# rahulaggarwal965/vslam

Measured on AMD Instinct MI355X. Metric: frame-pairs/sec (extract+match+RANSAC) @1280×720, 2k kp, 4096 hyp; 1/2/4/8 GPU, higher is better.
Workload: dtype u8/f32/f64; 1 GPU; C3: 1280x720, 2000 keypoints, 4096 hypotheses, batch 256 pairs per GPU, SURVEY 8(d) data: rotation + parallax, sub-pixel resampling, 40-45 % outlier matches; pairs_per_gpu=256, batches_in_flight=4

## Files before the change

vslam_amd/csrc/ransac_count.hip:

```cpp
#include "ransac_prune_tile.h"
#include "ransac_residual.h"

namespace {
using namespace vs_ransac;

constexpr int kCntHyps = 128;
constexpr int kCntWaves = 8;
constexpr int kCntQueue = 320;
constexpr int kCntLdsMatches = 4096;
constexpr int kScreenMatches = 128;
constexpr int kScreenHyps = 128;
constexpr int kRankThreads = 512;
constexpr int kPilotHyps = kRankThreads / 64;
constexpr int kCandMax = 8;
constexpr float kCntTinyDD = 0x1p-120f;
constexpr int kFcmpOGT = 2, kFcmpOLT = 4, kFcmpULT = 12;
constexpr int kCntRec = 12;
typedef __attribute__((address_space(3))) volatile uint32_t cnt_queue_t;
static_assert(VSLAM_MAX_KP <= 65536, "queue words keep the match index in 16 bits");

__host__ __device__ constexpr int cnt_pad(int n) { return (n + 255) & ~255; }
constexpr int kHeadUncertified = kVsHeadUncertified;
__device__ __forceinline__ float cnt_sum_rel(int adds) { return fmaxf(0x1p-18f, (float)(13 + adds) * 0x1p-24f); }

// ... 197 lines not shown
}

__global__ __launch_bounds__(kRankThreads) void ransac_rank_kernel(
    const float *__restrict__ xy1, const float *__restrict__ xy2, const int32_t *__restrict__ pairs,
    const int32_t *__restrict__ m_arr, int min_m, int kp_stride, int kp_pad, int hyp, float threshold,
    const float *__restrict__ hypF, int32_t *__restrict__ cbound, float *__restrict__ rk, float *__restrict__ cmax,
    unsigned long long *__restrict__ sfloor) {
    const int b = blockIdx.x, tid = threadIdx.x, lane = tid & 63;
    const int wave = __builtin_amdgcn_readfirstlane(tid >> 6);
    const int m = min(m_arr[b], kp_stride);
    if (m < min_m) return;
    __shared__ double s_psum[kPilotHyps];
    __shared__ unsigned long long s_bits[kPilotHyps][VSLAM_MAX_KP / 64];
    __shared__ int s_hist[kPilotHyps][kPilotHyps + 1], s_off[kPilotHyps][kPilotHyps + 1], s_pcount[kPilotHyps];
    const float2 *P1 = reinterpret_cast<const float2 *>(xy1) + (size_t)b * kp_stride;
    const float2 *P2 = reinterpret_cast<const float2 *>(xy2) + (size_t)b * kp_stride;
    const int2 *PR = reinterpret_cast<const int2 *>(pairs) + (size_t)b * kp_stride;
    const int npil = min(kPilotHyps, hyp);
    const int G = (m + 63) >> 6;

    if (wave < npil) {
        const int h = (int)(((long long)hyp * wave) / npil);
        ResidualF R;
        const float *src = hypF + ((size_t)b * hyp + h) * 9;
#pragma unroll
        for (int j = 0; j < 9; j++) R.f[j] = src[j];
        residual_prepare(R);
        int count = 0;
        double esum = 0;
        float c1 = 0.f, c2 = 0.f;
        for (int g0 = 0; g0 < G; g0 += 4) {
            int2 pr[4];
            float2 a[4], c[4];
#pragma unroll
            for (int u = 0; u < 4; u++) pr[u] = PR[min((g0 + u) * 64 + lane, m - 1)];
#pragma unroll
            for (int u = 0; u < 4; u++) {
                a[u] = P1[pr[u].x];
                c[u] = P2[pr[u].y];
            }
#pragma unroll
            for (int u = 0; u < 4; u++) {
                const float e = residual_e(R, make_float4(a[u].x, a[u].y, c[u].x, c[u].y), (double)c[u].x, (double)c[u].y);
                const unsigned long long in = __ballot((g0 + u) * 64 + lane < m && e <= threshold);
                count += __popcll(in);
                if ((g0 + u) * 64 + lane < m) esum += (double)e;
                if (lane == 0 && g0 + u < G) s_bits[wave][g0 + u] = in;
                c1 = fmaxf(c1, fmaxf(fabsf(a[u].x), fabsf(a[u].y)));
                c2 = fmaxf(c2, fmaxf(fabsf(c[u].x), fabsf(c[u].y)));
            }
        }
#pragma unroll
        for (int off = 32; off > 0; off >>= 1) esum += __shfl_xor(esum, off, 64);
        if (lane == 0) {
            s_pcount[wave] = count;
            s_psum[wave] = esum;
        }
        if (wave == 0) {
#pragma unroll
            for (int off = 32; off > 0; off >>= 1) {
                c1 = fmaxf(c1, __shfl_xor(c1, off, 64));
                c2 = fmaxf(c2, __shfl_xor(c2, off, 64));
            }
            if (lane == 0) {
                cmax[2 * b] = c1;
                cmax[2 * b + 1] = c2;
            }
        }
    }
    __syncthreads();

    const int gpw = (G + kPilotHyps - 1) / kPilotHyps;
    const int g_lo = min(G, wave * gpw), g_hi = min(G, g_lo + gpw);
    int hist[kPilotHyps + 1];
#pragma unroll
    for (int v = 0; v <= kPilotHyps; v++) hist[v] = 0;
    for (int g = g_lo; g < g_hi; g++) {
        const bool valid = g * 64 + lane < m;
        int key = 0;
        for (int w = 0; w < npil; w++) key += (int)((~s_bits[w][g] >> lane) & 1ull);
#pragma unroll
        for (int v = 0; v <= kPilotHyps; v++) hist[v] += __popcll(__ballot(valid && key == v));
    }
    if (lane == 0) {
#pragma unroll
        for (int v = 0; v <= kPilotHyps; v++) s_hist[wave][v] = hist[v];
    }
    __syncthreads();
    if (tid == 0) {
        int best = 0;
        for (int w = 0; w < npil; w++) best = max(best, s_pcount[w]);
        cbound[b] = best;
        if (sfloor) {
            double fl = -INFINITY;
            bool any_nan = false;
            for (int w = 0; w < npil; w++)
                if (s_pcount[w] == best) {
                    any_nan = any_nan || !(s_psum[w] == s_psum[w]);
                    if (s_psum[w] > fl) fl = s_psum[w];
                }
            const bool valid = best > 0 && !any_nan && fl > 0 && fl < 0x1p120;
            sfloor[b] = valid ? ((unsigned long long)(uint32_t)best << 32) | (unsigned long long)__float_as_uint((float)(fl * (1.0 - 0x1p-20))) : 0ull;
        }
        int run = 0;
        for (int v = kPilotHyps; v >= 0; v--)
            for (int w = 0; w < kPilotHyps; w++) {
                s_off[w][v] = run;
                run += s_hist[w][v];
            }
    }
    __syncthreads();
    int off[kPilotHyps + 1];
#pragma unroll
    for (int v = 0; v <= kPilotHyps; v++) off[v] = s_off[wave][v];
    float *r = rk + (size_t)b * 4 * kp_pad;
    for (int g = g_lo; g < g_hi; g++) {
        const int i = g * 64 + lane;
        const bool valid = i < m;
        int key = 0;
        for (int w = 0; w < npil; w++) key += (int)((~s_bits[w][g] >> lane) & 1ull);
        int pos = 0;
#pragma unroll
        for (int v = 0; v <= kPilotHyps; v++) {
            const unsigned long long bal = __ballot(valid && key == v);
            const int rank = (int)__builtin_amdgcn_mbcnt_hi((uint32_t)(bal >> 32), __builtin_amdgcn_mbcnt_lo((uint32_t)bal, 0u));
            if (key == v) pos = off[v] + rank;
            off[v] += __popcll(bal);
        }
        if (valid) {
            const int2 pr = PR[i];
            const float2 a = P1[pr.x], c = P2[pr.y];
            r[pos] = a.x;
            r[kp_pad + pos] = a.y;
            r[2 * kp_pad + pos] = c.x;
            r[3 * kp_pad + pos] = c.y;
        }
    }
    const int mpad = cnt_pad(m);
    if (m + tid < mpad) {
        const int2 pr = PR[m - 1];
        const float2 a = P1[pr.x], c = P2[pr.y];
        r[m + tid] = a.x;
        r[kp_pad + m + tid] = a.y;
        r[2 * kp_pad + m + tid] = c.x;
        r[3 * kp_pad + m + tid] = c.y;
    }
}

#ifdef VSLAM_EXPERIMENTS
#define VS_SCREEN_ROUTE_PARAM , int32_t *__restrict__ route_out
#else
#define VS_SCREEN_ROUTE_PARAM
#endif
__global__ __launch_bounds__(256) __attribute__((amdgpu_waves_per_eu(7, 7))) void ransac_screen_kernel(
    const float *__restrict__ rk, int kp_pad, const int32_t *__restrict__ m_arr, int min_m, int kp_stride, int hyp,
    float threshold, const float *__restrict__ hypF, const float *__restrict__ cmax, const int32_t *__restrict__ cbound,
    int32_t *__restrict__ pot0, int2 *__restrict__ head, float splus, int route VS_SCREEN_ROUTE_PARAM) {
    const int b = blockIdx.y, tid = threadIdx.x, lane = tid & 63;
    const int wave = __builtin_amdgcn_readfirstlane(tid >> 6);
    const int hbase = blockIdx.x * kScreenHyps;
    const int m = min(m_arr[b], kp_stride);
    const int bound_pilots = cbound[b];
#ifdef VSLAM_EXPERIMENTS
    if (route_out && blockIdx.x == 0 && tid == 0)
        route_out[b] = m < min_m ? -1 : (vs_head_on_certificate(m, bound_pilots, min(m, kScreenMatches), route) ? 1 : 0);
#endif
    if (m < min_m) return;
    if (vs_head_on_certificate(m, bound_pilots, min(m, kScreenMatches), route)) {
        static_assert(kScreenHyps == vs_prune::kPruneWaves * vs_prune::kPruneHyps && kScreenMatches <= vs_prune::kHeadTiles * vs_prune::kPruneTile,
                      "a wave of the screen is a wave of the prune tile");
        if (hbase + wave * 32 < hyp)
            vs_prune::head_on_certificate(rk, kp_pad, b, m, min(m, kScreenMatches), hbase + wave * 32, hyp, threshold, splus, hypF, cmax, pot0, head);
        return;
    }
    __shared__ __align__(16) float s_rec[kScreenHyps * kCntRec];
    if (tid < kScreenHyps) {
        const float *src = hypF + ((size_t)b * hyp + min(hbase + tid, hyp - 1)) * 9;
        float f[9];
#pragma unroll
        for (int k = 0; k < 9; k++) f[k] = src[k];
        const CntBand B = cnt_band(f, cmax[2 * b], cmax[2 * b + 1], threshold);
        cnt_store_record(s_rec + tid * kCntRec, f, B);
    }
    const int n0 = min(m, kScreenMatches);
    const float *r = rk + (size_t)b * 4 * kp_pad;
    const float2 x1 = *reinterpret_cast<const float2 *>(r + 2 * lane);
    const float2 y1 = *reinterpret_cast<const float2 *>(r + kp_pad + 2 * lane);
    const float2 x2 = *reinterpret_cast<const float2 *>(r + 2 * kp_pad + 2 * lane);
    const float2 y2 = *reinterpret_cast<const float2 *>(r + 3 * kp_pad + 2 * lane);
    v2f X1, Y1, X2, Y2;
    X1.x = x1.x; X1.y = x1.y; Y1.x = y1.x; Y1.y = y1.y;
    X2.x = x2.x; X2.y = x2.y; Y2.x = y2.x; Y2.y = y2.y;
    const unsigned long long va = __ballot(2 * lane < n0), vb = __ballot(2 * lane + 1 < n0);
    __syncthreads();
    int mine = 0;
    float mine_sum = 0.f;
    const bool odd1 = (lane & 1) != 0, odd2 = (lane & 2) != 0;
    const bool in_a = 2 * lane < n0, in_b = 2 * lane + 1 < n0;
    constexpr int kU = 4;
    static_assert(kU == 4, "the head sums are reduced four hypotheses at a time");
    for (int j = 0; j < 32; j += kU) {
        CntRec R[kU];
        v2f dd[kU], g[kU];
#pragma unroll
        for (int u = 0; u < kU; u++) cnt_load_record(R[u], s_rec, wave * 32 + j + u);
#pragma unroll
        for (int u = 0; u < kU; u++) g[u] = cnt_cheap(R[u], X1, Y1, X2, Y2, dd[u]);
        bool any_alive = false;
#pragma unroll
        for (int u = 0; u < kU; u++) {
            const unsigned long long oa = __builtin_amdgcn_fcmpf(g[u].x, R[u].hi, kFcmpOGT), ob = __builtin_amdgcn_fcmpf(g[u].y, R[u].hi, kFcmpOGT);
            const unsigned long long ia = __builtin_amdgcn_fcmpf(g[u].x, R[u].lo, kFcmpOLT), ib = __builtin_amdgcn_fcmpf(g[u].y, R[u].lo, kFcmpOLT);
            int p = __popcll(va & ~oa) + __popcll(vb & ~ob);
            int c = __popcll(va & ia) + __popcll(vb & ib);
            if (__builtin_amdgcn_fcmpf(fminf(dd[u].x, dd[u].y), kCntTinyDD, kFcmpULT) != 0ull) {
                p = n0;
                c = 0xFF;
            }
            mine = lane == j + u ? (p | (c << 8)) : mine;
            any_alive = any_alive || p + (m - n0) >= bound_pilots;
        }
        if (!any_alive) continue;
        float v[kU];
#pragma unroll
        for (int u = 0; u < kU; u++) v[u] = (in_a ? g[u].x : 0.f) + (in_b ? g[u].y : 0.f);
        const int z = 0;
        const float k01 = odd1 ? v[1] : v[0], t01 = odd1 ? v[0] : v[1], k23 = odd1 ? v[3] : v[2], t23 = odd1 ? v[2] : v[3];
        const float r01 = k01 + __int_as_float(__builtin_amdgcn_update_dpp(z, __float_as_int(t01), 0xB1, 0xF, 0xF, false));
        const float r23 = k23 + __int_as_float(__builtin_amdgcn_update_dpp(z, __float_as_int(t23), 0xB1, 0xF, 0xF, false));
        const float kk = odd2 ? r23 : r01, tt = odd2 ? r01 : r23;
        float r = kk + __int_as_float(__builtin_amdgcn_update_dpp(z, __float_as_int(tt), 0x4E, 0xF, 0xF, false));
        r += __int_as_float(__builtin_amdgcn_update_dpp(z, __float_as_int(r), 0x124, 0xF, 0xF, false));
        r += __int_as_float(__builtin_amdgcn_update_dpp(z, __float_as_int(r), 0x128, 0xF, 0xF, false));
        r += __shfl_xor(r, 16, 64);
        r += __shfl_xor(r, 32, 64);
        mine_sum = (lane >> 2) == (j >> 2) ? r : mine_sum;
    }
    const int h = hbase + wave * 32 + lane;
    if (lane < 32 && h < hyp) {
        const int c = mine >> 8;
        pot0[(size_t)b * hyp + h] = mine & 0xFF;
        head[(size_t)b * hyp + h] = make_int2(c == 0xFF ? kHeadUncertified : c, __float_as_int(mine_sum));
    }
}

__global__ __launch_bounds__(64 * kCandMax) void ransac_cand_kernel(
    const float *__restrict__ rk, int kp_pad, const int32_t *__restrict__ m_arr, int min_m, int kp_stride, int hyp,
    float threshold, const float *__restrict__ hypF, const int32_t *__restrict__ pot0, int by_sum,
    int32_t *__restrict__ cbound, unsigned long long *__restrict__ sfloor) {
    const int b = blockIdx.x, tid = threadIdx.x, lane = tid & 63;
    const int wave = __builtin_amdgcn_readfirstlane(tid >> 6);
    const int m = min(m_arr[b], kp_stride);
    if (m < min_m) return;
    __shared__ int s_max[kCandMax], s_l0[kCandMax][kCandMax], s_l1[kCandMax][kCandMax], s_n0[kCandMax], s_n1[kCandMax];
    __shared__ int s_cand[kCandMax], s_nc;
    const int32_t *P = pot0 + (size_t)b * hyp;
    int mx = -1;
    for (int i = tid; i < hyp; i += 64 * kCandMax) mx = max(mx, P[i]);
#pragma unroll
    for (int off = 32; off > 0; off >>= 1) mx = max(mx, __shfl_xor(mx, off, 64));
    if (lane == 0) s_max[wave] = mx;
    __syncthreads();
    mx = s_max[0];
    for (int w = 1; w < kCandMax; w++) mx = max(mx, s_max[w]);
    const int per = (hyp + kCandMax - 1) / kCandMax;
    const int lo = min(hyp, wave * per), hi = min(hyp, lo + per);
    int n0 = 0, n1 = 0;
    __shared__ int s_samp[kCandMax][32];
    int nsamp = 0;
    for (int i0 = lo; i0 < hi && ((by_sum && nsamp < 32) || n0 < kCandMax || n1 < kCandMax); i0 += 64) {
        const int i = i0 + lane;
        const int v = i < hi ? P[i] : -2;
        unsigned long long b0 = __ballot(v == mx), b1 = __ballot(v == mx - 1);
        if (by_sum) {
            const int rs = nsamp + __popcll(b0 & ((1ull << lane) - 1ull));
            if (v == mx && rs < 32) s_samp[wave][rs] = i;
            nsamp = min(32, nsamp + (int)__popcll(b0));
        }
        const int r0 = n0 + __popcll(b0 & ((1ull << lane) - 1ull)), r1 = n1 + __popcll(b1 & ((1ull << lane) - 1ull));
        if (v == mx && r0 < kCandMax) s_l0[wave][r0] = i;
        if (v == mx - 1 && r1 < kCandMax) s_l1[wave][r1] = i;
        n0 = min(kCandMax, n0 + __popcll(b0));
        n1 = min(kCandMax, n1 + __popcll(b1));
    }
    if (by_sum && nsamp > 1) {
        const int n128 = min(m, kScreenMatches);
        const float *r = rk + (size_t)b * 4 * kp_pad;
        const float2 x1 = *reinterpret_cast<const float2 *>(r + 2 * lane), y1 = *reinterpret_cast<const float2 *>(r + kp_pad + 2 * lane);
        const float2 x2 = *reinterpret_cast<const float2 *>(r + 2 * kp_pad + 2 * lane), y2 = *reinterpret_cast<const float2 *>(r + 3 * kp_pad + 2 * lane);
        v2f X1, Y1, X2, Y2;
        X1.x = x1.x; X1.y = x1.y; Y1.x = y1.x; Y1.y = y1.y;
        X2.x = x2.x; X2.y = x2.y; Y2.x = y2.x; Y2.y = y2.y;
        float fl[9];
        {
            const int hs = s_samp[wave][lane < nsamp ? lane : 0];
            const float *src = hypF + ((size_t)b * hyp + hs) * 9;
#pragma unroll
            for (int k = 0; k < 9; k++) fl[k] = src[k];
        }
        float best_s = -INFINITY;
        int best_i = -1;
        for (int j = 0; j < nsamp; j++) {
            CntRec R;
#pragma unroll
            for (int k = 0; k < 9; k++) R.f[k] = __int_as_float(__builtin_amdgcn_readlane(__float_as_int(fl[k]), j));
            v2f dd;
            const v2f g = cnt_cheap(R, X1, Y1, X2, Y2, dd);
            const float part = wave_sum_to_lane63((2 * lane < n128 ? g.x : 0.f) + (2 * lane + 1 < n128 ? g.y : 0.f));
            const float tot = __int_as_float(__builtin_amdgcn_readlane(__float_as_int(part), 63));
            if (tot > best_s) {
                best_s = tot;
                best_i = s_samp[wave][j];
            }
        }
        if (lane == 0 && best_i >= 0 && n0 > 0) {
            const int old = s_l0[wave][0];
            for (int k = 1; k < n0; k++)
                if (s_l0[wave][k] == best_i) s_l0[wave][k] = old;
            s_l0[wave][0] = best_i;
        }
    }
    if (lane == 0) {
        s_n0[wave] = n0;
        s_n1[wave] = n1;
    }
// ... 158 lines not shown
            if (lane == 0) knext = atomicAdd(&s_next, 1);
            int hh;
            {
                int kk = k, w = 0;
                while (w + 1 < kListWaves && kk >= s_nlist[w]) kk -= s_nlist[w++];
                hh = s_list[w * 64 + kk];
            }
            bound = max(bound, *(__attribute__((address_space(3))) const volatile int *)&s_bound);
            CntRec R;
            cnt_load_record(R, s_rec, hh);
            const int word = ZERO ? 0 : s_state[hh] >> 2;
            const int head_cnt = ZERO ? 0 : *(__attribute__((address_space(3))) const volatile int *)&s_cnt[hh];
            float head_sum = ZERO ? 0.f : s_part[hh];
            int cnt = 0, pot = word & 0xFFFF, seen = org;
            bool dropped = false, unk = false;
            v2f acc;
            acc.x = 0.f;
            acc.y = 0.f;
            for (int s = 0;; s++) {
                if (s >= nsub && (ZERO || s > nsub || !(word & kHeadMine))) break;
                const bool hd = !ZERO && s == nsub;
                const int pot_walk = pot;
                const int ix = (hd ? 0 : org + s * 256) + 4 * lane;
                const int il = min(ix, mpad - 4);
                const float4 X1 = *reinterpret_cast<const float4 *>(cx1 + il), Y1 = *reinterpret_cast<const float4 *>(cy1 + il);
                const float4 X2 = *reinterpret_cast<const float4 *>(cx2 + il), Y2 = *reinterpret_cast<const float4 *>(cy2 + il);
                if (hd || (s == nsub - 1 && part)) {
                    cnt_sub_block<true>(R, X1, Y1, X2, Y2, ix, hh, lane, hd ? n0 : m, cnt, q, qn, acc, s_unk, pot, unk);
                    seen += hd ? 0 : (m - org) & 255;
                } else {
                    cnt_sub_block<false>(R, X1, Y1, X2, Y2, ix, hh, lane, m, cnt, q, qn, acc, s_unk, pot, unk);
                    seen += 256;
                }
                while (qn >= 64) {
                    cnt_drain(q, qn - 64, 64, lane, s_rec, s_cnt, cx1, cy1, cx2, cy2, threshold);
                    qn -= 64;
                }
                if (hd) {
                    head_sum = 0.f;
                    pot = pot_walk;
                    break;
                }
                if (pot + (m - seen) < bound) {
                    dropped = true;
                    break;
                }
                if (seen < m && bound == floor_count && pot + (m - seen) == bound && !unk && R.beta >= 0.f && !(word & kHeadNoSum)) {
                    const float S = head_sum + __int_as_float(__builtin_amdgcn_readlane(__float_as_int(wave_sum_to_lane63(acc.x + acc.y)), 63));
                    const float ns = (float)seen;
                    const float err = (2.02f * R.beta * sqrtf(ns * S) + ns * R.beta * R.beta + sum_rel * S) * 1.0001f;
                    const float upper = ((S + err) + threshold * (float)(m - seen)) * 1.0001f;
                    if (upper < floor_sum * 0.9999f) {
                        dropped = true;
                        break;
                    }
                }
            }
            if (dropped) {
#ifdef VSLAM_EXPERIMENTS
                if (lane == 0) s_state[hh] = 2 | (seen << 2);
#else
                if (lane == 0) s_state[hh] = 2;
#endif
            } else {
                const float part_sum = head_sum + wave_sum_to_lane63(acc.x + acc.y);
                bool beaten = false;
                if (bound == floor_count && pot == bound && !unk && R.beta >= 0.f) {
                    const float S = __int_as_float(__builtin_amdgcn_readlane(__float_as_int(part_sum), 63));
                    const float ns = (float)m;
                    const float err = (2.02f * R.beta * sqrtf(ns * S) + ns * R.beta * R.beta + sum_rel * S) * 1.0001f;
                    beaten = (S + err) * 1.0001f < floor_sum * 0.9999f;
                }
                if (lane == 63) s_part[hh] = part_sum;
                const int certain = head_cnt + cnt;
                if (beaten) {
#ifdef VSLAM_EXPERIMENTS
                    if (lane == 0) s_state[hh] = 2 | (seen << 2);
#else
                    if (lane == 0) s_state[hh] = 2;
#endif
                } else if (lane == 0) {
                    if (cnt) atomicAdd(&s_cnt[hh], cnt);
                    if (certain > bound) {
                        atomicMax(&s_bound, certain);
                        atomicMax(&cbound[b], certain);
                    }
                }
                if (!beaten) bound = max(bound, certain);
            }
            k = __builtin_amdgcn_readfirstlane(knext);
        }
        if (qn > 0) cnt_drain(q, 0, qn, lane, s_rec, s_cnt, cx1, cy1, cx2, cy2, threshold);
    }
    __syncthreads();
    if (tid < nh) {
        const int st = s_state[tid] & 3;
        hyp_count[out] = st == 1 ? s_cnt[tid] : -1;
        int nan_bits = 0x7FC00000;
#ifdef VSLAM_EXPERIMENTS
        if (exit_payload && st != 1) nan_bits |= st == 2 ? min(s_state[tid] >> 2, 0x3FFFFF) : 0x3FFFFF;
#endif
        hyp_sum[out] = __int_as_float(nan_bits);
        const float S = st == 1 ? s_part[tid] : 0.f;
        float err = INFINITY;
        if (st == 1 && my_ok && !s_unk[tid]) {
            const double Sd = (double)S;
            const double rel = (double)cnt_sum_rel(2 * ((m - (ZERO ? 0 : n0) + 255) >> 8) + 9);
            err = (float)((2.02 * my_beta * sqrt((double)m * Sd) + (double)m * my_beta * my_beta + rel * Sd) * (1.0 + 0x1p-20));
        }
        reinterpret_cast<float2 *>(approx)[out] = make_float2(S, err);
    }
}

}

int vs_launch_ransac_count(vslam_ctx *ctx, const float *xy1, const float *xy2, const int32_t *pairs, const int32_t *m,
                           const float *hypF, int batch, int kp_stride, int hyp, float threshold, int32_t *hyp_count,
                           float *hyp_sum, float *approx) {
    const int min_m = ctx->ransac_min_matches;
    int rc;
    int32_t *cbound = nullptr, *pot0 = nullptr;
    float *rk = nullptr, *cmax = nullptr;
    const int kp_pad = cnt_pad(kp_stride);
    if ((rc = vs_arena_get(ctx, "ransac.cbound", sizeof(int32_t) * (size_t)batch, (void **)&cbound))) return rc;
    unsigned long long *sfloor = nullptr;
    if ((rc = vs_arena_get(ctx, "ransac.sfloor", sizeof(unsigned long long) * (size_t)batch, (void **)&sfloor))) return rc;
    static const bool no_sum_rule = VS_EXPERIMENT_ENV("VSLAM_RANSAC_NO_SUM_RULE") != nullptr;
    const bool from_zero = VS_EXPERIMENT_ENV("VSLAM_RANSAC_COUNT_FROM_ZERO") != nullptr;
#ifdef VSLAM_EXPERIMENTS
    const int exit_payload = VS_EXPERIMENT_ENV("VSLAM_RANSAC_COUNT_EXIT_PAYLOAD") != nullptr ? 1 : 0;
#endif
    int2 *head = nullptr;
    if ((rc = vs_arena_get(ctx, "ransac.head", sizeof(int2) * (size_t)batch * hyp, (void **)&head))) return rc;
    const unsigned long long *use_floor = no_sum_rule ? nullptr : sfloor;
    if ((rc = vs_arena_get(ctx, "ransac.pot0", sizeof(int32_t) * (size_t)batch * hyp, (void **)&pot0))) return rc;
    if ((rc = vs_arena_get(ctx, "ransac.rk", sizeof(float) * 4 * (size_t)kp_pad * batch, (void **)&rk))) return rc;
    if ((rc = vs_arena_get(ctx, "ransac.cmax", sizeof(float) * 2 * (size_t)batch, (void **)&cmax))) return rc;
    {
        VsProfScope ps(ctx, "ransac_rank_kernel");
        ransac_rank_kernel<<<batch, kRankThreads, 0, ctx->stream>>>(xy1, xy2, pairs, m, min_m, kp_stride, kp_pad, hyp, threshold, hypF,
                                                                    cbound, rk, cmax, sfloor);
    }
    int route = -1;
    if (const char *e = VS_EXPERIMENT_ENV("VSLAM_RANSAC_HEAD_ROUTE")) route = atoi(e) ? 1 : 0;
#ifdef VSLAM_EXPERIMENTS
    int32_t *route_out = nullptr, *pot0_out = nullptr;
    if ((rc = vs_arena_get(ctx, "ransac.head_route", sizeof(int32_t) * (size_t)batch, (void **)&route_out))) return rc;
    if ((rc = vs_arena_get(ctx, "ransac.head_pot0", sizeof(int32_t) * (size_t)batch * hyp, (void **)&pot0_out))) return rc;
#endif
    {
        VsProfScope ps(ctx, "ransac_screen_kernel");
        dim3 grid(vs_div_up(hyp, kScreenHyps), batch);
#ifdef VSLAM_EXPERIMENTS
        ransac_screen_kernel<<<grid, 256, 0, ctx->stream>>>(rk, kp_pad, m, min_m, kp_stride, hyp, threshold, hypF, cmax, cbound, pot0, head,
                                                            pc_splus(threshold), route, route_out);
#else
        ransac_screen_kernel<<<grid, 256, 0, ctx->stream>>>(rk, kp_pad, m, min_m, kp_stride, hyp, threshold, hypF, cmax, cbound, pot0, head,
                                                            pc_splus(threshold), route);
#endif
    }
#ifdef VSLAM_EXPERIMENTS
    VS_HIP(ctx, hipMemcpyAsync(pot0_out, pot0, sizeof(int32_t) * (size_t)batch * hyp, hipMemcpyDeviceToDevice, ctx->stream));
#endif
    {
        VsProfScope ps(ctx, "ransac_cand_kernel");
        ransac_cand_kernel<<<batch, 64 * kCandMax, 0, ctx->stream>>>(rk, kp_pad, m, min_m, kp_stride, hyp, threshold, hypF, pot0,
                                                                     no_sum_rule ? 0 : 1, cbound, sfloor);
    }
    if ((rc = vs_launch_ransac_prune(ctx, rk, kp_pad, m, min_m, kp_stride, hyp, threshold, hypF, cmax, cbound, pot0, batch, kScreenMatches)))
        return rc;
    if (int arc = vs_aux_job_point(ctx, 4)) return arc;
    {
        VsProfScope ps(ctx, "ransac_count_kernel");
        const bool lds = kp_pad <= kCntLdsMatches;
        const size_t dyn = (lds ? sizeof(float) * 4 * (size_t)kp_pad : 0) + sizeof(uint32_t) * kCntQueue * kCntWaves;
        const size_t dyn_max = sizeof(float) * 4 * kCntLdsMatches + sizeof(uint32_t) * kCntQueue * kCntWaves;
        dim3 grid(vs_div_up(hyp, kCntHyps), batch);
#ifdef VSLAM_EXPERIMENTS
        if (from_zero) {
            if (dyn > 32 * 1024 && (rc = vs_allow_dynamic_lds(ctx, ransac_count_kernel<true, true>, "ransac_count_from_zero", dyn_max)))
                return rc;
            if (lds)
                ransac_count_kernel<true, true><<<grid, 64 * kCntWaves, dyn, ctx->stream>>>(
                    rk, kp_pad, m, min_m, kp_stride, hyp, threshold, hypF, pot0, head, cmax, hyp_count, hyp_sum, approx, cbound,
                    use_floor VS_CNT_PAYLOAD_ARG);
            else
                ransac_count_kernel<false, true><<<grid, 64 * kCntWaves, dyn, ctx->stream>>>(
                    rk, kp_pad, m, min_m, kp_stride, hyp, threshold, hypF, pot0, head, cmax, hyp_count, hyp_sum, approx, cbound,
                    use_floor VS_CNT_PAYLOAD_ARG);
            return VSLAM_OK;
        }
#endif
        (void)from_zero;
        if (dyn > 32 * 1024 &&
            (rc = vs_allow_dynamic_lds(ctx, ransac_count_kernel<true, false>, "ransac_count", dyn_max)))
            return rc;
        if (lds)
            ransac_count_kernel<true, false><<<grid, 64 * kCntWaves, dyn, ctx->stream>>>(
                rk, kp_pad, m, min_m, kp_stride, hyp, threshold, hypF, pot0, head, cmax, hyp_count, hyp_sum, approx, cbound,
                    use_floor VS_CNT_PAYLOAD_ARG);
        else
            ransac_count_kernel<false, false><<<grid, 64 * kCntWaves, dyn, ctx->stream>>>(
                rk, kp_pad, m, min_m, kp_stride, hyp, threshold, hypF, pot0, head, cmax, hyp_count, hyp_sum, approx, cbound,
                    use_floor VS_CNT_PAYLOAD_ARG);
    }
    return VSLAM_OK;
}
```

vslam_amd/csrc/ransac_prune.hip:

```cpp
#include "ransac_prune_tile.h"

namespace {
using namespace vs_prune;

constexpr int kPruneStep = 2;

#ifdef VSLAM_EXPERIMENTS
#define VS_PRUNE_X_PARAM , int32_t *__restrict__ x_out
#else
#define VS_PRUNE_X_PARAM
#endif

__global__ __launch_bounds__(64 * kPruneWaves) void ransac_prune_mfma_kernel(
    const float *__restrict__ rk, int kp_pad, const int32_t *__restrict__ m_arr, int min_m, int kp_stride, int hyp, float threshold,
    float splus, const float *__restrict__ hypF, const float *__restrict__ cmax, const int32_t *__restrict__ cbound, int32_t *__restrict__ pot0,
    int n_head, int gate VS_PRUNE_X_PARAM) {
    const int b = blockIdx.y, lane = threadIdx.x & 63, col = lane & 31;
    const bool half = lane >= 32;
    const int wave = __builtin_amdgcn_readfirstlane(threadIdx.x >> 6);
    const int m = min(m_arr[b], kp_stride);
    const int bound = cbound[b];
    if (m < min_m) return;
    const int n0 = min(m, n_head);
    const int hbase = (blockIdx.x * kPruneWaves + wave) * kPruneHyps;
    if (m <= n0 || hbase >= hyp) return;
    if (gate && m - bound + 1 <= n0) return;

    const int h = hbase + col;
    const size_t hi = (size_t)b * hyp + min(h, hyp - 1);
    const int behind = m - n0;
    const int lim = pot0[hi] + behind - bound;
    bool live0 = h < hyp && lim >= 0 && lim < behind;
    if (__ballot(live0) == 0ull) return;
    float f[9];
#pragma unroll
    for (int k = 0; k < 9; k++) f[k] = hypF[hi * 9 + k];
    const float c = pc_margin(f, cmax[2 * b], cmax[2 * b + 1], threshold, splus);
    live0 = live0 && c < INFINITY;
    if (__ballot(live0) == 0ull) return;
    const PruneA A = prune_operands(f, half);
    float cr[16];
#pragma unroll
    for (int r = 0; r < 16; r++) cr[r] = __shfl(c, half ? prune_row(r, 1) : prune_row(r, 0), 64);

    const float *r1 = rk + (size_t)b * 4 * kp_pad, *r2 = r1 + kp_pad, *r3 = r2 + kp_pad, *r4 = r3 + kp_pad;
    int X[kPruneHyps], L[kPruneHyps];
#pragma unroll
    for (int i = 0; i < kPruneHyps; i++) {
        X[i] = 0;
        L[i] = __builtin_amdgcn_readlane(live0 ? lim : -1, i);
    }
    const int end = m;
    for (int base = n0; base < end; base += kPruneStep * kPruneTile) {
        float x1[kPruneStep], y1[kPruneStep], x2[kPruneStep], y2[kPruneStep];
#pragma unroll
        for (int t = 0; t < kPruneStep; t++) {
            const int j = min(base + t * kPruneTile + col, m - 1);
            x1[t] = r1[j];
            y1[t] = r2[j];
            x2[t] = r3[j];
            y2[t] = r4[j];
        }
#pragma unroll
        for (int t = 0; t < kPruneStep; t++) {
            v16f n, a0;
            prune_tile(A, half, x1[t], y1[t], x2[t], y2[t], n, a0);
            const unsigned long long valid = __ballot(base + t * kPruneTile + col < end);
#pragma unroll
            for (int r = 0; r < 16; r++) {
                const unsigned long long miss =
                    __builtin_amdgcn_fcmpf(fabsf(n[r]), fmaf(splus, fabsf(a0[r]), cr[r]), kPruneOGT) & valid;
                X[prune_row(r, 0)] += __popc((uint32_t)miss);
                X[prune_row(r, 1)] += __popc((uint32_t)(miss >> 32));
            }
        }
        int top = -1;
#pragma unroll
        for (int i = 0; i < kPruneHyps; i++) top = max(top, X[i] <= L[i] ? X[i] : -1);
        const int seen = min(base + kPruneStep * kPruneTile, end) - n0;
        if (top < 0 || 2 * top < seen) break;
    }
    int xv = 0;
#pragma unroll
    for (int i = 0; i < kPruneHyps; i++) xv = col == i ? X[i] : xv;
    if (!half && h < hyp) {
        if (live0 && xv > lim) pot0[hi] = -behind - 1;
#ifdef VSLAM_EXPERIMENTS
        if (x_out) x_out[hi] = xv;
#endif
    }
}

#ifdef VSLAM_EXPERIMENTS
__global__ __launch_bounds__(64) void ransac_prune_tile_kernel(const float *__restrict__ F, const float *__restrict__ xy,
                                                               float *__restrict__ n_out, float *__restrict__ a0_out) {
    const int lane = threadIdx.x, col = lane & 31;
    const bool half = lane >= 32;
    float f[9];
#pragma unroll
    for (int k = 0; k < 9; k++) f[k] = F[col * 9 + k];
    const PruneA A = prune_operands(f, half);
    v16f n, a0;
    prune_tile(A, half, xy[col], xy[32 + col], xy[64 + col], xy[96 + col], n, a0);
#pragma unroll
    for (int r = 0; r < 16; r++) {
        const int row = half ? prune_row(r, 1) : prune_row(r, 0);
        n_out[row * 32 + col] = n[r];
        a0_out[row * 32 + col] = a0[r];
    }
}
#endif

}

int vs_launch_ransac_prune(vslam_ctx *ctx, const float *rk, int kp_pad, const int32_t *m, int min_m, int kp_stride, int hyp,
                           float threshold, const float *hypF, const float *cmax, const int32_t *cbound, int32_t *pot0, int batch,
                           int n_head) {
    if (VS_EXPERIMENT_ENV("VSLAM_RANSAC_NO_PRUNE") != nullptr) return VSLAM_OK;
    int gate = 1;
    if (const char *e = VS_EXPERIMENT_ENV("VSLAM_RANSAC_PRUNE_GATE")) gate = atoi(e);
#ifdef VSLAM_EXPERIMENTS
    int32_t *x_out = nullptr;
    if (int rc = vs_arena_get(ctx, "ransac.prune_x", sizeof(int32_t) * (size_t)batch * hyp, (void **)&x_out)) return rc;
    VS_HIP(ctx, hipMemsetAsync(x_out, 0, sizeof(int32_t) * (size_t)batch * hyp, ctx->stream));
#endif
    VsProfScope ps(ctx, "ransac_prune_kernel");
    dim3 grid(vs_div_up(hyp, kPruneWaves * kPruneHyps), batch);
#ifdef VSLAM_EXPERIMENTS
    ransac_prune_mfma_kernel<<<grid, 64 * kPruneWaves, 0, ctx->stream>>>(rk, kp_pad, m, min_m, kp_stride, hyp, threshold, pc_splus(threshold), hypF, cmax,
                                                                         cbound, pot0, n_head, gate, x_out);
#else
    ransac_prune_mfma_kernel<<<grid, 64 * kPruneWaves, 0, ctx->stream>>>(rk, kp_pad, m, min_m, kp_stride, hyp, threshold, pc_splus(threshold), hypF, cmax,
                                                                         cbound, pot0, n_head, gate);
#endif
    return VSLAM_OK;
}

#ifdef VSLAM_EXPERIMENTS
extern "C" {
int vslam_debug_ransac_prune_x(vslam_ctx *ctx, int32_t *d_out, int batch, int hyp) {
    if (!ctx) return VSLAM_ERR_INVALID;
    VS_REQUIRE(ctx, d_out && batch > 0 && hyp > 0 && vs_ptr_bits(d_out) % 4 == 0, VSLAM_ERR_INVALID);
    const size_t bytes = sizeof(int32_t) * (size_t)batch * hyp;
    const auto it = ctx->arena.find("ransac.prune_x");
    VS_REQUIRE(ctx, it != ctx->arena.end() && it->second.bytes >= bytes, VSLAM_ERR_INVALID);
    VS_HIP(ctx, hipMemcpyAsync(d_out, it->second.ptr, bytes, hipMemcpyDeviceToDevice, ctx->stream));
    return VSLAM_OK;
}
int vslam_debug_ransac_head(vslam_ctx *ctx, int32_t *d_pot0, int32_t *d_route, int batch, int hyp) {
    if (!ctx) return VSLAM_ERR_INVALID;
    VS_REQUIRE(ctx, d_pot0 && d_route && batch > 0 && hyp > 0 && vs_ptr_bits(d_pot0, d_route) % 4 == 0, VSLAM_ERR_INVALID);
    const size_t bytes = sizeof(int32_t) * (size_t)batch * hyp;
    const auto ip = ctx->arena.find("ransac.head_pot0"), ir = ctx->arena.find("ransac.head_route");
    VS_REQUIRE(ctx, ip != ctx->arena.end() && ip->second.bytes >= bytes, VSLAM_ERR_INVALID);
    VS_REQUIRE(ctx, ir != ctx->arena.end() && ir->second.bytes >= sizeof(int32_t) * (size_t)batch, VSLAM_ERR_INVALID);
    VS_HIP(ctx, hipMemcpyAsync(d_pot0, ip->second.ptr, bytes, hipMemcpyDeviceToDevice, ctx->stream));
    VS_HIP(ctx, hipMemcpyAsync(d_route, ir->second.ptr, sizeof(int32_t) * (size_t)batch, hipMemcpyDeviceToDevice, ctx->stream));
    return VSLAM_OK;
}
int vslam_debug_ransac_prune_tile(vslam_ctx *ctx, const float *d_F, const float *d_xy, float *d_n, float *d_a0) {
    if (!ctx) return VSLAM_ERR_INVALID;
    VS_REQUIRE(ctx, d_F && d_xy && d_n && d_a0 && vs_ptr_bits(d_F, d_xy, d_n, d_a0) % 4 == 0, VSLAM_ERR_INVALID);
    ransac_prune_tile_kernel<<<1, 64, 0, ctx->stream>>>(d_F, d_xy, d_n, d_a0);
    return VSLAM_OK;
}
}
#endif
```

vslam_amd/csrc/ransac_prune_tile.h:

```cpp
#pragma once

#include "ransac_prune_cert.h"
#include "ransac_residual.h"

namespace vs_prune {

typedef float v16f __attribute__((ext_vector_type(16)));
constexpr int kPruneWaves = 4;
constexpr int kPruneHyps = 32;
constexpr int kPruneTile = 32;
constexpr int kPruneOGT = 2;

__host__ __device__ constexpr int prune_row(int r, int half) { return (r & 3) + 8 * (r >> 2) + 4 * half; }

struct PruneA {
    float n[5], d[2];
};
__device__ __forceinline__ PruneA prune_operands(const float *f, bool half) {
    PruneA A;
#pragma unroll
    for (int s = 0; s < 4; s++) A.n[s] = half ? f[2 * s + 1] : f[2 * s];
    A.n[4] = half ? 0.f : f[8];
    A.d[0] = half ? f[1] : f[0];
    A.d[1] = half ? 0.f : f[2];
    return A;
}

__device__ __forceinline__ void prune_tile(const PruneA &A, bool half, float x1, float y1, float x2, float y2, v16f &n, v16f &a0) {
    const float p = x2 * (half ? y1 : x1);
    const float q = y2 * (half ? x1 : y1);
    const float b1 = half ? q : x2, b2 = half ? y2 : q, b3 = half ? y1 : x1, b4 = half ? 0.f : 1.f;
    v16f z;
#pragma unroll
    for (int r = 0; r < 16; r++) z[r] = 0.f;
    n = __builtin_amdgcn_mfma_f32_32x32x2f32(A.n[0], p, z, 0, 0, 0);
    n = __builtin_amdgcn_mfma_f32_32x32x2f32(A.n[1], b1, n, 0, 0, 0);
    n = __builtin_amdgcn_mfma_f32_32x32x2f32(A.n[2], b2, n, 0, 0, 0);
    n = __builtin_amdgcn_mfma_f32_32x32x2f32(A.n[3], b3, n, 0, 0, 0);
    n = __builtin_amdgcn_mfma_f32_32x32x2f32(A.n[4], b4, n, 0, 0, 0);
    a0 = __builtin_amdgcn_mfma_f32_32x32x2f32(A.d[0], b3, z, 0, 0, 0);
    a0 = __builtin_amdgcn_mfma_f32_32x32x2f32(A.d[1], b4, a0, 0, 0, 0);
}

constexpr int kHeadTiles = 4;
__device__ __forceinline__ void head_on_certificate(const float *__restrict__ rk, int kp_pad, int b, int m, int n0, int hbase, int hyp,
                                                    float threshold, float splus, const float *__restrict__ hypF,
                                                    const float *__restrict__ cmax, int32_t *__restrict__ pot0, int2 *__restrict__ head) {
    const int lane = threadIdx.x & 63, col = lane & 31;
    const bool half = lane >= 32;
    const int h = hbase + col;
    const size_t hi = (size_t)b * hyp + min(h, hyp - 1);
    float f[9];
#pragma unroll
    for (int k = 0; k < 9; k++) f[k] = hypF[hi * 9 + k];
    const float c = pc_margin(f, cmax[2 * b], cmax[2 * b + 1], threshold, splus);
    const PruneA A = prune_operands(f, half);
    float cr[16];
#pragma unroll
    for (int r = 0; r < 16; r++) cr[r] = __shfl(c, half ? prune_row(r, 1) : prune_row(r, 0), 64);

    const float *r1 = rk + (size_t)b * 4 * kp_pad, *r2 = r1 + kp_pad, *r3 = r2 + kp_pad, *r4 = r3 + kp_pad;
    float x1[kHeadTiles], y1[kHeadTiles], x2[kHeadTiles], y2[kHeadTiles];
#pragma unroll
    for (int t = 0; t < kHeadTiles; t++) {
        const int j = min(t * kPruneTile + col, m - 1);
        x1[t] = r1[j];
        y1[t] = r2[j];
        x2[t] = r3[j];
        y2[t] = r4[j];
    }
    int X[kPruneHyps];
#pragma unroll
    for (int i = 0; i < kPruneHyps; i++) X[i] = 0;
#pragma unroll
    for (int t = 0; t < kHeadTiles; t++) {
        if (t * kPruneTile >= n0) break;
        v16f n, a0;
        prune_tile(A, half, x1[t], y1[t], x2[t], y2[t], n, a0);
        const unsigned long long valid = __ballot(t * kPruneTile + col < n0);
#pragma unroll
        for (int r = 0; r < 16; r++) {
            const unsigned long long miss =
                __builtin_amdgcn_fcmpf(fabsf(n[r]), fmaf(splus, fabsf(a0[r]), cr[r]), kPruneOGT) & valid;
            X[prune_row(r, 0)] += __popc((uint32_t)miss);
            X[prune_row(r, 1)] += __popc((uint32_t)(miss >> 32));
        }
    }
    int xv = 0;
#pragma unroll
    for (int i = 0; i < kPruneHyps; i++) xv = col == i ? X[i] : xv;
    if (!half && h < hyp) {
        pot0[hi] = n0 - xv;
        head[hi] = make_int2(kVsHeadUncertified, 0);
    }
}

}
```

Before: 105,300 frame-pairs/s.

## Transpose prune MFMA operands so each lane owns one hypothesis and counts locally

```diff
diff --git a/vslam_amd/csrc/ransac_count.hip b/vslam_amd/csrc/ransac_count.hip
--- a/vslam_amd/csrc/ransac_count.hip
+++ b/vslam_amd/csrc/ransac_count.hip
@@ -373,6 +373,7 @@
 #else
 #define VS_SCREEN_ROUTE_PARAM
 #endif
+template <bool kRows>
 __global__ __launch_bounds__(256) __attribute__((amdgpu_waves_per_eu(7, 7))) void ransac_screen_kernel(
     const float *__restrict__ rk, int kp_pad, const int32_t *__restrict__ m_arr, int min_m, int kp_stride, int hyp,
     float threshold, const float *__restrict__ hypF, const float *__restrict__ cmax, const int32_t *__restrict__ cbound,
@@ -390,8 +391,14 @@
     if (vs_head_on_certificate(m, bound_pilots, min(m, kScreenMatches), route)) {
         static_assert(kScreenHyps == vs_prune::kPruneWaves * vs_prune::kPruneHyps && kScreenMatches <= vs_prune::kHeadTiles * vs_prune::kPruneTile,
                       "a wave of the screen is a wave of the prune tile");
-        if (hbase + wave * 32 < hyp)
-            vs_prune::head_on_certificate(rk, kp_pad, b, m, min(m, kScreenMatches), hbase + wave * 32, hyp, threshold, splus, hypF, cmax, pot0, head);
+        if (hbase + wave * 32 < hyp) {
+#ifdef VSLAM_EXPERIMENTS
+            if constexpr (kRows)
+                vs_prune::head_on_certificate_rows(rk, kp_pad, b, m, min(m, kScreenMatches), hbase + wave * 32, hyp, threshold, splus, hypF, cmax, pot0, head);
+            else
+#endif
+                vs_prune::head_on_certificate(rk, kp_pad, b, m, min(m, kScreenMatches), hbase + wave * 32, hyp, threshold, splus, hypF, cmax, pot0, head);
+        }
         return;
     }
     __shared__ __align__(16) float s_rec[kScreenHyps * kCntRec];
@@ -856,11 +863,15 @@
         VsProfScope ps(ctx, "ransac_screen_kernel");
         dim3 grid(vs_div_up(hyp, kScreenHyps), batch);
 #ifdef VSLAM_EXPERIMENTS
-        ransac_screen_kernel<<<grid, 256, 0, ctx->stream>>>(rk, kp_pad, m, min_m, kp_stride, hyp, threshold, hypF, cmax, cbound, pot0, head,
-                                                            pc_splus(threshold), route, route_out);
+        if (vs_prune_rows_form())
+            ransac_screen_kernel<true><<<grid, 256, 0, ctx->stream>>>(rk, kp_pad, m, min_m, kp_stride, hyp, threshold, hypF, cmax, cbound, pot0, head,
+                                                                      pc_splus(threshold), route, route_out);
+        else
+            ransac_screen_kernel<false><<<grid, 256, 0, ctx->stream>>>(rk, kp_pad, m, min_m, kp_stride, hyp, threshold, hypF, cmax, cbound, pot0, head,
+                                                                       pc_splus(threshold), route, route_out);
 #else
-        ransac_screen_kernel<<<grid, 256, 0, ctx->stream>>>(rk, kp_pad, m, min_m, kp_stride, hyp, threshold, hypF, cmax, cbound, pot0, head,
-                                                            pc_splus(threshold), route);
+        ransac_screen_kernel<false><<<grid, 256, 0, ctx->stream>>>(rk, kp_pad, m, min_m, kp_stride, hyp, threshold, hypF, cmax, cbound, pot0, head,
+                                                                   pc_splus(threshold), route);
 #endif
     }
 #ifdef VSLAM_EXPERIMENTS
diff --git a/vslam_amd/csrc/ransac_prune.hip b/vslam_amd/csrc/ransac_prune.hip
--- a/vslam_amd/csrc/ransac_prune.hip
+++ b/vslam_amd/csrc/ransac_prune.hip
@@ -11,7 +11,7 @@
 #define VS_PRUNE_X_PARAM
 #endif
 
-__global__ __launch_bounds__(64 * kPruneWaves) void ransac_prune_mfma_kernel(
+__global__ __launch_bounds__(64 * kPruneWaves) __attribute__((amdgpu_waves_per_eu(4))) void ransac_prune_mfma_kernel(
     const float *__restrict__ rk, int kp_pad, const int32_t *__restrict__ m_arr, int min_m, int kp_stride, int hyp, float threshold,
     float splus, const float *__restrict__ hypF, const float *__restrict__ cmax, const int32_t *__restrict__ cbound, int32_t *__restrict__ pot0,
     int n_head, int gate VS_PRUNE_X_PARAM) {
@@ -39,17 +39,11 @@
     live0 = live0 && c < INFINITY;
     if (__ballot(live0) == 0ull) return;
     const PruneA A = prune_operands(f, half);
-    float cr[16];
-#pragma unroll
-    for (int r = 0; r < 16; r++) cr[r] = __shfl(c, half ? prune_row(r, 1) : prune_row(r, 0), 64);
 
     const float *r1 = rk + (size_t)b * 4 * kp_pad, *r2 = r1 + kp_pad, *r3 = r2 + kp_pad, *r4 = r3 + kp_pad;
-    int X[kPruneHyps], L[kPruneHyps];
-#pragma unroll
-    for (int i = 0; i < kPruneHyps; i++) {
-        X[i] = 0;
-        L[i] = __builtin_amdgcn_readlane(live0 ? lim : -1, i);
-    }
+    const int row4 = half ? 4 : 0;
+    int cnt = 0;
+    int xv = 0;
     const int end = m;
     for (int base = n0; base < end; base += kPruneStep * kPruneTile) {
         float x1[kPruneStep], y1[kPruneStep], x2[kPruneStep], y2[kPruneStep];
@@ -61,10 +55,89 @@
             x2[t] = r3[j];
             y2[t] = r4[j];
         }
+        if (base + kPruneStep * kPruneTile <= end) {
+#pragma unroll
+            for (int t = 0; t < kPruneStep; t++) {
+                v16f n, a0;
+                prune_tile(A, half, x1[t], y1[t], x2[t], y2[t], n, a0);
+                cnt = prune_count(n, a0, splus, c, cnt);
+            }
+        } else {
+#pragma unroll
+            for (int t = 0; t < kPruneStep; t++) {
+                v16f n, a0;
+                prune_tile(A, half, x1[t], y1[t], x2[t], y2[t], n, a0);
+                cnt = prune_count(n, a0, splus, c, cnt, end - (base + t * kPruneTile) - row4);
+            }
+        }
+        xv = cnt + __shfl_xor(cnt, 32, 64);
+        const int seen = min(base + kPruneStep * kPruneTile, end) - n0;
+        const bool alive = live0 && xv <= lim;
+        if (__ballot(alive && 2 * xv >= seen) == 0ull) break;
+    }
+    if (!half && h < hyp) {
+        if (live0 && xv > lim) pot0[hi] = -behind - 1;
+#ifdef VSLAM_EXPERIMENTS
+        if (x_out) x_out[hi] = xv;
+#endif
+    }
+}
+
+#ifdef VSLAM_EXPERIMENTS
+__global__ __launch_bounds__(64 * kPruneWaves) void ransac_prune_rows_kernel(
+    const float *__restrict__ rk, int kp_pad, const int32_t *__restrict__ m_arr, int min_m, int kp_stride, int hyp, float threshold,
+    float splus, const float *__restrict__ hypF, const float *__restrict__ cmax, const int32_t *__restrict__ cbound, int32_t *__restrict__ pot0,
+    int n_head, int gate, int32_t *__restrict__ x_out) {
+    const int b = blockIdx.y, lane = threadIdx.x & 63, col = lane & 31;
+    const bool half = lane >= 32;
+    const int wave = __builtin_amdgcn_readfirstlane(threadIdx.x >> 6);
+    const int m = min(m_arr[b], kp_stride);
+    const int bound = cbound[b];
+    if (m < min_m) return;
+    const int n0 = min(m, n_head);
+    const int hbase = (blockIdx.x * kPruneWaves + wave) * kPruneHyps;
+    if (m <= n0 || hbase >= hyp) return;
+    if (gate && m - bound + 1 <= n0) return;
+
+    const int h = hbase + col;
+    const size_t hi = (size_t)b * hyp + min(h, hyp - 1);
+    const int behind = m - n0;
+    const int lim = pot0[hi] + behind - bound;
+    bool live0 = h < hyp && lim >= 0 && lim < behind;
+    if (__ballot(live0) == 0ull) return;
+    float f[9];
+#pragma unroll
+    for (int k = 0; k < 9; k++) f[k] = hypF[hi * 9 + k];
+    const float c = pc_margin(f, cmax[2 * b], cmax[2 * b + 1], threshold, splus);
+    live0 = live0 && c < INFINITY;
+    if (__ballot(live0) == 0ull) return;
+    const PruneA A = prune_operands(f, half);
+    float cr[16];
+#pragma unroll
+    for (int r = 0; r < 16; r++) cr[r] = __shfl(c, half ? prune_row(r, 1) : prune_row(r, 0), 64);
+
+    const float *r1 = rk + (size_t)b * 4 * kp_pad, *r2 = r1 + kp_pad, *r3 = r2 + kp_pad, *r4 = r3 + kp_pad;
+    int X[kPruneHyps], L[kPruneHyps];
+#pragma unroll
+    for (int i = 0; i < kPruneHyps; i++) {
+        X[i] = 0;
+        L[i] = __builtin_amdgcn_readlane(live0 ? lim : -1, i);
+    }
+    const int end = m;
+    for (int base = n0; base < end; base += kPruneStep * kPruneTile) {
+        float x1[kPruneStep], y1[kPruneStep], x2[kPruneStep], y2[kPruneStep];
+#pragma unroll
+        for (int t = 0; t < kPruneStep; t++) {
+            const int j = min(base + t * kPruneTile + col, m - 1);
+            x1[t] = r1[j];
+            y1[t] = r2[j];
+            x2[t] = r3[j];
+            y2[t] = r4[j];
+        }
 #pragma unroll
         for (int t = 0; t < kPruneStep; t++) {
             v16f n, a0;
-            prune_tile(A, half, x1[t], y1[t], x2[t], y2[t], n, a0);
+            prune_tile_rows(A, half, x1[t], y1[t], x2[t], y2[t], n, a0);
             const unsigned long long valid = __ballot(base + t * kPruneTile + col < end);
 #pragma unroll
             for (int r = 0; r < 16; r++) {
@@ -85,11 +158,10 @@
     for (int i = 0; i < kPruneHyps; i++) xv = col == i ? X[i] : xv;
     if (!half && h < hyp) {
         if (live0 && xv > lim) pot0[hi] = -behind - 1;
-#ifdef VSLAM_EXPERIMENTS
         if (x_out) x_out[hi] = xv;
-#endif
-    }
-}
+    }
+}
+#endif
 
 #ifdef VSLAM_EXPERIMENTS
 __global__ __launch_bounds__(64) void ransac_prune_tile_kernel(const float *__restrict__ F, const float *__restrict__ xy,
@@ -105,8 +177,8 @@
 #pragma unroll
     for (int r = 0; r < 16; r++) {
         const int row = half ? prune_row(r, 1) : prune_row(r, 0);
-        n_out[row * 32 + col] = n[r];
-        a0_out[row * 32 + col] = a0[r];
+        n_out[col * 32 + row] = n[r];
+        a0_out[col * 32 + row] = a0[r];
     }
 }
 #endif
@@ -127,8 +199,12 @@
     VsProfScope ps(ctx, "ransac_prune_kernel");
     dim3 grid(vs_div_up(hyp, kPruneWaves * kPruneHyps), batch);
 #ifdef VSLAM_EXPERIMENTS
-    ransac_prune_mfma_kernel<<<grid, 64 * kPruneWaves, 0, ctx->stream>>>(rk, kp_pad, m, min_m, kp_stride, hyp, threshold, pc_splus(threshold), hypF, cmax,
-                                                                         cbound, pot0, n_head, gate, x_out);
+    if (vs_prune_rows_form())
+        ransac_prune_rows_kernel<<<grid, 64 * kPruneWaves, 0, ctx->stream>>>(rk, kp_pad, m, min_m, kp_stride, hyp, threshold, pc_splus(threshold), hypF,
+                                                                             cmax, cbound, pot0, n_head, gate, x_out);
+    else
+        ransac_prune_mfma_kernel<<<grid, 64 * kPruneWaves, 0, ctx->stream>>>(rk, kp_pad, m, min_m, kp_stride, hyp, threshold, pc_splus(threshold), hypF,
+                                                                             cmax, cbound, pot0, n_head, gate, x_out);
 #else
     ransac_prune_mfma_kernel<<<grid, 64 * kPruneWaves, 0, ctx->stream>>>(rk, kp_pad, m, min_m, kp_stride, hyp, threshold, pc_splus(threshold), hypF, cmax,
                                                                          cbound, pot0, n_head, gate);
diff --git a/vslam_amd/csrc/ransac_prune_tile.h b/vslam_amd/csrc/ransac_prune_tile.h
--- a/vslam_amd/csrc/ransac_prune_tile.h
+++ b/vslam_amd/csrc/ransac_prune_tile.h
@@ -33,6 +33,77 @@
     v16f z;
 #pragma unroll
     for (int r = 0; r < 16; r++) z[r] = 0.f;
+    n = __builtin_amdgcn_mfma_f32_32x32x2f32(p, A.n[0], z, 0, 0, 0);
+    n = __builtin_amdgcn_mfma_f32_32x32x2f32(b1, A.n[1], n, 0, 0, 0);
+    n = __builtin_amdgcn_mfma_f32_32x32x2f32(b2, A.n[2], n, 0, 0, 0);
+    n = __builtin_amdgcn_mfma_f32_32x32x2f32(b3, A.n[3], n, 0, 0, 0);
+    n = __builtin_amdgcn_mfma_f32_32x32x2f32(b4, A.n[4], n, 0, 0, 0);
+    a0 = __builtin_amdgcn_mfma_f32_32x32x2f32(b3, A.d[0], z, 0, 0, 0);
+    a0 = __builtin_amdgcn_mfma_f32_32x32x2f32(b4, A.d[1], a0, 0, 0, 0);
+}
+
+__device__ __forceinline__ int prune_count(const v16f &n, const v16f &a0, float splus, float c, int cnt) {
+#pragma unroll
+    for (int r = 0; r < 16; r++) cnt += fabsf(n[r]) > fmaf(splus, fabsf(a0[r]), c) ? 1 : 0;
+    return cnt;
+}
+__device__ __forceinline__ int prune_count(const v16f &n, const v16f &a0, float splus, float c, int cnt, int rem) {
+#pragma unroll
+    for (int r = 0; r < 16; r++)
+        cnt += (prune_row(r, 0) < rem && fabsf(n[r]) > fmaf(splus, fabsf(a0[r]), c)) ? 1 : 0;
+    return cnt;
+}
+
+constexpr int kHeadTiles = 4;
+__device__ __forceinline__ void head_on_certificate(const float *__restrict__ rk, int kp_pad, int b, int m, int n0, int hbase, int hyp,
+                                                    float threshold, float splus, const float *__restrict__ hypF,
+                                                    const float *__restrict__ cmax, int32_t *__restrict__ pot0, int2 *__restrict__ head) {
+    const int lane = threadIdx.x & 63, col = lane & 31;
+    const bool half = lane >= 32;
+    const int h = hbase + col;
+    const size_t hi = (size_t)b * hyp + min(h, hyp - 1);
+    float f[9];
+#pragma unroll
+    for (int k = 0; k < 9; k++) f[k] = hypF[hi * 9 + k];
+    const float c = pc_margin(f, cmax[2 * b], cmax[2 * b + 1], threshold, splus);
+    const PruneA A = prune_operands(f, half);
+
+    const float *r1 = rk + (size_t)b * 4 * kp_pad, *r2 = r1 + kp_pad, *r3 = r2 + kp_pad, *r4 = r3 + kp_pad;
+    float x1[kHeadTiles], y1[kHeadTiles], x2[kHeadTiles], y2[kHeadTiles];
+#pragma unroll
+    for (int t = 0; t < kHeadTiles; t++) {
+        const int j = min(t * kPruneTile + col, m - 1);
+        x1[t] = r1[j];
+        y1[t] = r2[j];
+        x2[t] = r3[j];
+        y2[t] = r4[j];
+    }
+    int cnt = 0;
+#pragma unroll
+    for (int t = 0; t < kHeadTiles; t++) {
+        if (t * kPruneTile >= n0) break;
+        v16f n, a0;
+        prune_tile(A, half, x1[t], y1[t], x2[t], y2[t], n, a0);
+        if ((t + 1) * kPruneTile <= n0)
+            cnt = prune_count(n, a0, splus, c, cnt);
+        else
+            cnt = prune_count(n, a0, splus, c, cnt, n0 - t * kPruneTile - (half ? 4 : 0));
+    }
+    const int xv = cnt + __shfl_xor(cnt, 32, 64);
+    if (!half && h < hyp) {
+        pot0[hi] = n0 - xv;
+        head[hi] = make_int2(kVsHeadUncertified, 0);
+    }
+}
+
+#ifdef VSLAM_EXPERIMENTS
+__device__ __forceinline__ void prune_tile_rows(const PruneA &A, bool half, float x1, float y1, float x2, float y2, v16f &n, v16f &a0) {
+    const float p = x2 * (half ? y1 : x1);
+    const float q = y2 * (half ? x1 : y1);
+    const float b1 = half ? q : x2, b2 = half ? y2 : q, b3 = half ? y1 : x1, b4 = half ? 0.f : 1.f;
+    v16f z;
+#pragma unroll
+    for (int r = 0; r < 16; r++) z[r] = 0.f;
     n = __builtin_amdgcn_mfma_f32_32x32x2f32(A.n[0], p, z, 0, 0, 0);
     n = __builtin_amdgcn_mfma_f32_32x32x2f32(A.n[1], b1, n, 0, 0, 0);
     n = __builtin_amdgcn_mfma_f32_32x32x2f32(A.n[2], b2, n, 0, 0, 0);
@@ -42,10 +113,9 @@
     a0 = __builtin_amdgcn_mfma_f32_32x32x2f32(A.d[1], b4, a0, 0, 0, 0);
 }
 
-constexpr int kHeadTiles = 4;
-__device__ __forceinline__ void head_on_certificate(const float *__restrict__ rk, int kp_pad, int b, int m, int n0, int hbase, int hyp,
-                                                    float threshold, float splus, const float *__restrict__ hypF,
-                                                    const float *__restrict__ cmax, int32_t *__restrict__ pot0, int2 *__restrict__ head) {
+__device__ __forceinline__ void head_on_certificate_rows(const float *__restrict__ rk, int kp_pad, int b, int m, int n0, int hbase, int hyp,
+                                                         float threshold, float splus, const float *__restrict__ hypF,
+                                                         const float *__restrict__ cmax, int32_t *__restrict__ pot0, int2 *__restrict__ head) {
     const int lane = threadIdx.x & 63, col = lane & 31;
     const bool half = lane >= 32;
     const int h = hbase + col;
@@ -76,7 +146,7 @@
     for (int t = 0; t < kHeadTiles; t++) {
         if (t * kPruneTile >= n0) break;
         v16f n, a0;
-        prune_tile(A, half, x1[t], y1[t], x2[t], y2[t], n, a0);
+        prune_tile_rows(A, half, x1[t], y1[t], x2[t], y2[t], n, a0);
         const unsigned long long valid = __ballot(t * kPruneTile + col < n0);
 #pragma unroll
         for (int r = 0; r < 16; r++) {
@@ -94,5 +164,11 @@
         head[hi] = make_int2(kVsHeadUncertified, 0);
     }
 }
+#endif
 
 }
+
+inline bool vs_prune_rows_form() {
+    const char *e = VS_EXPERIMENT_ENV("VSLAM_RANSAC_PRUNE_ROWS");
+    return e != nullptr && atoi(e) != 0;
+}
```

Result: faster. 107,100 frame-pairs/s, median of 6 (+1.7%).
